# JettHuang/jet-pbrt

Hardware: AMD Instinct MI355X
Metric: Msamples/sec (whole node) + per-pixel L2 vs CPU ref, cornell_box 1024spp (higher is better)
Workload: dtype f32

## Files before the change

### jet-pbrt_amd/__init__.py

```python
import ctypes as C
import os

PKG_DIR = os.path.dirname(os.path.abspath(__file__))
REPO_DIR = os.path.dirname(PKG_DIR)
HIP_LIB_PATH = os.environ.get("JETPBRT_AMD_LIB") or os.path.join(PKG_DIR, "csrc", "libjetpbrt_amd.so")
HOST_LIB_PATH = os.path.join(PKG_DIR, "host", "libjetpbrt_host.so")
CLI_PATH = os.path.join(PKG_DIR, "host", "jetpbrt")

JP_MAT_PARAM_STRIDE = 16
JP_SAMPLER_STOCK_MT19937, JP_SAMPLER_COUNTER, JP_SAMPLER_DEBUG = 0, 1, 2
JP_OK = 0

_fp = C.POINTER(C.c_float)
_ip = C.POINTER(C.c_int32)


class JpCamera(C.Structure):
    _fields_ = [("pos", C.c_float * 3), ("front", C.c_float * 3), ("right", C.c_float * 3), ("up", C.c_float * 3),
                ("res_x", C.c_float), ("res_y", C.c_float)]


class JpScene(C.Structure):
    _fields_ = [
        ("camera", JpCamera),
# ... 1053 lines not shown
        v = tri_vn if isinstance(tri_vn, JpVertexNormals) else vertex_normals(tri_vn)
        self._check(self.lib.jp_set_vertex_normals(self.h, C.byref(v)))

    def normal_info(self):
        i = JpNormalInfo()
        i.struct_bytes = C.sizeof(JpNormalInfo)
        self._check(self.lib.jp_get_normal_info(self.h, C.byref(i)))
        return i

    def set_normal_maps(self, maps):
        self._check(self.lib.jp_set_normal_maps(self.h, None if maps is None else C.byref(maps)))

    def normal_map_info(self):
        i = JpNormalMapInfo()
        i.struct_bytes = C.sizeof(JpNormalMapInfo)
        self._check(self.lib.jp_get_normal_map_info(self.h, C.byref(i)))
        return i

    def set_texture_sampling(self, sampling):
        self._check(self.lib.jp_set_texture_sampling(self.h, None if sampling is None else C.byref(sampling)))

    def texture_sampling_info(self):
        i = JpTexSamplingInfo()
        i.struct_bytes = C.sizeof(JpTexSamplingInfo)
        self._check(self.lib.jp_get_texture_sampling_info(self.h, C.byref(i)))
        return i

    def shading_normal(self, origin, direction, tmin, tmax):
        import numpy as np
        n = origin.shape[0]
        o = np.ascontiguousarray(origin, np.float32); d = np.ascontiguousarray(direction, np.float32)
        t0 = np.ascontiguousarray(tmin, np.float32); t1 = np.ascontiguousarray(tmax, np.float32)
        prim = np.zeros(n, np.int32); ng = np.zeros((n, 3), np.float32); ns = np.zeros((n, 3), np.float32)
        p = lambda a: a.ctypes.data_as(C.c_void_p)
        self._check(self.lib.jp_shading_normal(self.h, n, p(o), p(d), p(t0), p(t1), p(prim), p(ng), p(ns)))
        return prim, ng, ns

    def synchronize(self):
        self._check(self.lib.jp_synchronize(self.h))

    def set_profiling(self, on):
        self._check(self.lib.jp_set_profiling(self.h, 1 if on else 0))

    def counters(self):
        c = JpCounters()
        self._check(self.lib.jp_get_counters(self.h, C.byref(c)))
        return c

    def build_info(self):
        b = JpBuildInfo()
        self._check(self.lib.jp_get_build_info(self.h, C.byref(b)))
        return b

    def read_table(self, which):
        return _read_table(lambda out, cap, n: self.lib.jp_read_scene_table(self.h, _table_index(which), out, cap, n))

    def tree_info(self):
        i = JpTreeInfo()
        i.struct_bytes = C.sizeof(JpTreeInfo)
        self._check(self.lib.jp_get_tree_info(self.h, C.byref(i)))
        return i

    def trace(self, origin, direction, tmin, tmax):
        import numpy as np
        n = origin.shape[0]
        o = np.ascontiguousarray(origin, np.float32); d = np.ascontiguousarray(direction, np.float32)
        t0 = np.ascontiguousarray(tmin, np.float32); t1 = np.ascontiguousarray(tmax, np.float32)
        hit = np.zeros(n, np.int32); t = np.zeros(n, np.float32); prim = np.zeros(n, np.int32); nrm = np.zeros((n, 3), np.float32)
        p = lambda a: a.ctypes.data_as(C.c_void_p)
        self._check(self.lib.jp_trace(self.h, n, p(o), p(d), p(t0), p(t1), p(hit), p(t), p(prim), p(nrm)))
        return hit, t, prim, nrm

    def occluded(self, origin, direction, tmin, tmax):
        import numpy as np
        n = origin.shape[0]
        o = np.ascontiguousarray(origin, np.float32); d = np.ascontiguousarray(direction, np.float32)
        t0 = np.ascontiguousarray(tmin, np.float32); t1 = np.ascontiguousarray(tmax, np.float32)
        occ = np.zeros(n, np.int32); walk = C.c_int32(-1)
        p = lambda a: a.ctypes.data_as(C.c_void_p)
        self._check(self.lib.jp_occluded(self.h, n, p(o), p(d), p(t0), p(t1), p(occ), C.byref(walk)))
        return occ, int(walk.value)

    def bsdf(self, desc, normal, wo, wi, u):
        import numpy as np
        n = normal.shape[0]
        a = [np.ascontiguousarray(x, np.float32) for x in (normal, wo, wi, u)]
        out = dict(f=np.zeros((n, 3), np.float32), pdf=np.zeros(n, np.float32), sf=np.zeros((n, 3), np.float32), swi=np.zeros((n, 3), np.float32),
                   spdf=np.zeros(n, np.float32), sflags=np.zeros(n, np.int32))
        p = lambda x: x.ctypes.data_as(C.c_void_p)
        self._check(self.lib.jp_bsdf(self.h, C.byref(desc), n, p(a[0]), p(a[1]), p(a[2]), p(a[3]), p(out["f"]), p(out["pdf"]), p(out["sf"]), p(out["swi"]), p(out["spdf"]), p(out["sflags"])))
        return out

    def close(self):
        if self.h:
            self.lib.jp_destroy_context(self.h)
            self.h = C.c_void_p()

    def __del__(self):
        try:
            self.close()
        except Exception:
            pass


from . import scenes
from . import distributed
# ... 1 lines not shown
```

### jet-pbrt_amd/csrc/jp_device.h

```cpp
#pragma once
#include <hip/hip_runtime.h>
#include <stdint.h>
#include "jetpbrt_amd.h"
#include "jp_counter_rng.h"

#define JP_BLOCK 256
#define JP_STACK_DEPTH 32

namespace jp
{
struct V3 { float x, y, z; };
__device__ __forceinline__ V3 mk(float x, float y, float z) { V3 v; v.x = x; v.y = y; v.z = z; return v; }
__device__ __forceinline__ V3 operator+(V3 a, V3 b) { return mk(a.x + b.x, a.y + b.y, a.z + b.z); }
__device__ __forceinline__ V3 operator-(V3 a, V3 b) { return mk(a.x - b.x, a.y - b.y, a.z - b.z); }
__device__ __forceinline__ V3 operator-(V3 a) { return mk(-a.x, -a.y, -a.z); }
__device__ __forceinline__ V3 operator*(V3 a, float s) { return mk(a.x * s, a.y * s, a.z * s); }
__device__ __forceinline__ V3 operator*(float s, V3 a) { return mk(a.x * s, a.y * s, a.z * s); }
__device__ __forceinline__ V3 operator/(V3 a, float s) { return mk(a.x / s, a.y / s, a.z / s); }
__device__ __forceinline__ V3 cmul(V3 a, V3 b) { return mk(a.x * b.x, a.y * b.y, a.z * b.z); }
__device__ __forceinline__ V3 cdiv(V3 a, V3 b) { return mk(a.x / b.x, a.y / b.y, a.z / b.z); }
__device__ __forceinline__ V3 splat(float v) { return mk(v, v, v); }
__device__ __forceinline__ V3 csqrt(V3 a) { return mk(sqrtf(a.x), sqrtf(a.y), sqrtf(a.z)); }
__device__ __forceinline__ float dot(V3 a, V3 b) { return a.x * b.x + a.y * b.y + a.z * b.z; }
__device__ __forceinline__ float len2(V3 a) { return a.x * a.x + a.y * a.y + a.z * a.z; }
// ... 253 lines not shown
	    : "+v"(mask), "=&s"(saved) : "v"(a), "v"(b), "s"(bits) : "vcc", "scc");
}

template <bool kInfTmax>
__device__ __forceinline__ unsigned int flat_boxes_lean(const float4* flat_g, int n_flat, V3 o, V3 d, float tmin, float tmax)
{
	ConstFPtr flat = (ConstFPtr)flat_g;
	const float ix = __builtin_amdgcn_rcpf(d.x), iy = __builtin_amdgcn_rcpf(d.y), iz = __builtin_amdgcn_rcpf(d.z);
	unsigned int mask = 0;
	#define JP_FLAT_BOX(i) \
	{ \
		const float x0 = (flat[8 * (i) + 0] - o.x) * ix, x1 = (flat[8 * (i) + 4] - o.x) * ix; \
		const float y0 = (flat[8 * (i) + 1] - o.y) * iy, y1 = (flat[8 * (i) + 5] - o.y) * iy; \
		const float z0 = (flat[8 * (i) + 2] - o.z) * iz, z1 = (flat[8 * (i) + 6] - o.z) * iz; \
		const float tn = fmaxf(fmaxf(fminf(x0, x1), fminf(y0, y1)), fmaxf(fminf(z0, z1), tmin)); \
		const float fxy = fminf(fmaxf(x0, x1), fmaxf(y0, y1)), fz = fmaxf(z0, z1); \
		const float tf = kInfTmax ? fminf(fxy, fz) : fminf(fxy, fminf(fz, tmax)); \
		or_bits_if_le(mask, tn, tf * 1.000002f, __float_as_uint(flat[8 * (i) + 3])); \
	}
	int i0 = 0;
	for (; i0 + 4 <= n_flat; i0 += 4)
	{
		#pragma unroll
		for (int u = 0; u < 4; u++) JP_FLAT_BOX(i0 + u)
	}
	for (; i0 < n_flat; i0++) JP_FLAT_BOX(i0)
	#undef JP_FLAT_BOX
	return mask;
}

template <bool kAnyHit, bool k64, int kS, typename F = FeatAll, typename PrimPtr>
__device__ __forceinline__ int flat_prims(typename FlatMask<k64>::type mask, PrimPtr prims, V3 o, V3 d, float tmin, float& tmax)
{
	int hit = -1;
#ifdef JP_DBG_FLAT_P1ONLY
	mask = mask == (typename FlatMask<k64>::type)0x12345677u ? 1u : 0u;
#endif
	while (mask)
	{
		const int p = (k64 ? __ffsll((unsigned long long)mask) : __ffs((int)mask)) - 1;
		mask &= mask - 1;
		if (prim_hit<kS, F>(prims, p, o, d, tmin, tmax)) { hit = p; if (kAnyHit) return hit; }
	}
	return hit;
}

template <bool kAnyHit, int kS, typename F = FeatAll, bool kInfTmax = false, typename PrimPtr>
__device__ __forceinline__ int traverse_flat(const float4* flat_g, int n_flat, int n_prims, PrimPtr prims, V3 o, V3 d, float tmin, float& tmax)
{
	if constexpr (!F::curved)
		if (n_prims <= 32) return flat_prims<kAnyHit, false, kS, F>(flat_boxes_lean<kInfTmax>(flat_g, n_flat, o, d, tmin, tmax), prims, o, d, tmin, tmax);
	if (n_prims > 32) return flat_prims<kAnyHit, true, kS, F>(flat_boxes<true>(flat_g, n_flat, o, d, tmin, tmax), prims, o, d, tmin, tmax);
	return flat_prims<kAnyHit, false, kS, F>(flat_boxes<false>(flat_g, n_flat, o, d, tmin, tmax), prims, o, d, tmin, tmax);
}

template <bool kAnyHit, typename PrimPtr>
__device__ __forceinline__ int traverse_wide(const uint4* __restrict__ wide, PrimPtr prims, V3 o, V3 d, float tmin, float& tmax, unsigned int* stack)
{
	const float ix = 1.0f / d.x, iy = 1.0f / d.y, iz = 1.0f / d.z;
	const unsigned int octinv = 7u - ((d.x < 0 ? 1u : 0u) | (d.y < 0 ? 2u : 0u) | (d.z < 0 ? 4u : 0u));
	unsigned int ngx = 0, ngy = 0x80000000u;
	int hit = -1, sp = 0;
	for (;;)
	{
		unsigned int tgx = 0, tgy = 0;
		if (ngy > 0x00ffffffu)
		{
			const unsigned int bit = 31u - (unsigned int)__clz((int)ngy);
			ngy &= ~(1u << bit);
			if (ngy > 0x00ffffffu) { stack[(2 * sp) * JP_BLOCK] = ngx; stack[(2 * sp + 1) * JP_BLOCK] = ngy; sp++; }
			const unsigned int slot = (bit - 24u) ^ octinv;
			const unsigned int rel = (unsigned int)__popc(ngy & 0xffu & ~(0xffffffffu << slot));
			const unsigned int idx = ngx + rel;
			const uint4 q0 = wide[5 * idx + 0], q1 = wide[5 * idx + 1], q2 = wide[5 * idx + 2], q3 = wide[5 * idx + 3], q4 = wide[5 * idx + 4];
			const float sx = __uint_as_float(((q0.w & 0xffu) ) << 23), sy = __uint_as_float(((q0.w >> 8) & 0xffu) << 23), sz = __uint_as_float(((q0.w >> 16) & 0xffu) << 23);
			const float px = __uint_as_float(q0.x) - o.x, py = __uint_as_float(q0.y) - o.y, pz = __uint_as_float(q0.z) - o.z;
			unsigned int hm = 0;
			#pragma unroll
			for (int i = 0; i < 8; i++)
			{
				const int sh = 8 * (i & 3);
				const unsigned int m = ((i < 4 ? q1.z : q1.w) >> sh) & 0xffu;
				const float lx = (float)(((i < 4 ? q2.x : q2.y) >> sh) & 0xffu), ly = (float)(((i < 4 ? q2.z : q2.w) >> sh) & 0xffu), lz = (float)(((i < 4 ? q3.x : q3.y) >> sh) & 0xffu);
				const float hx = (float)(((i < 4 ? q3.z : q3.w) >> sh) & 0xffu), hy = (float)(((i < 4 ? q4.x : q4.y) >> sh) & 0xffu), hz = (float)(((i < 4 ? q4.z : q4.w) >> sh) & 0xffu);
				const float x0 = fmaf(lx, sx, px) * ix, x1 = fmaf(hx, sx, px) * ix;
				const float y0 = fmaf(ly, sy, py) * iy, y1 = fmaf(hy, sy, py) * iy;
				const float z0 = fmaf(lz, sz, pz) * iz, z1 = fmaf(hz, sz, pz) * iz;
				const float tn = fmaxf(fmaxf(fminf(x0, x1), fminf(y0, y1)), fmaxf(fminf(z0, z1), tmin));
				const float tf = fminf(fminf(fmaxf(x0, x1), fmaxf(y0, y1)), fminf(fmaxf(z0, z1), tmax));
				if (m != 0u && tn <= tf * 1.000002f)
				{
					const bool inner = (m & 0x18u) == 0x18u;
					const unsigned int bits = inner ? 1u : (m >> 5), at = inner ? 24u + ((m & 7u) ^ octinv) : (m & 31u);
					hm |= bits << at;
				}
			}
			ngx = q1.x; ngy = (hm & 0xff000000u) | (q0.w >> 24);
			tgx = q1.y; tgy = hm & 0x00ffffffu;
		}
		while (tgy)
		{
			const int j = __ffs((int)tgy) - 1;
			tgy &= tgy - 1;
			if (prim_hit<4>(prims, (int)tgx + j, o, d, tmin, tmax)) { hit = (int)tgx + j; if (kAnyHit) return hit; }
		}
		if (ngy <= 0x00ffffffu)
// ... 287 lines not shown
```

### jet-pbrt_amd/csrc/jp_kernels.hip

```cpp
#include "jp_common.h"
#include "jp_tex.h"
#include "jp_normals.h"
#include "jp_normal_map.h"
#include "jp_env.h"
#include "jp_mis.h"
#include "jp_lens.h"
#include "jp_xbsdf.h"
#include "jp_film.h"

#include <cstdio>
#include <cstring>
#include <string>
#include <vector>
#include <algorithm>
#include <cmath>
#include <mutex>
#include <thread>
#include "jp_devmem.h"
#include "jp_lbvh.h"
#include "jp_ploc.h"

struct NoLens {};
template <bool kLens> struct LensArg { typedef NoLens type; };
template <> struct LensArg<true> { typedef JpLensPlan type; };
// ... 692 lines not shown
	{
		const unsigned int e = rbase + j;
#ifdef JP_TRAV_TIMING
		JP_TT(1);
		asm volatile("s_waitcnt vmcnt(0)" ::: "memory");
		JP_TT(2);
#endif
		const float4 so = so_n; float4 sd = sd_n;
		if (j + JP_BLOCK < E) { so_n = q.sh_o[e + JP_BLOCK]; sd_n = q.sh_d[e + JP_BLOCK]; }
		const int packed = __float_as_int(so.w);
		const int slot = packed & ((1 << rc.slot_bits) - 1), n = (int)((unsigned int)packed >> rc.slot_bits);
		if (n == 0) continue;
		bool any = false;
		const float4 L = q.lacc[slot];
		V3 a = mk(L.x, L.y, L.z);
		for (int k = 0; k < n; k++)
		{
			const float4 c4 = q.sh_c[(size_t)k * q.cap + e];
			float tmax = sd.w;
			const V3 dir = xyz(sd);
			if (k + 1 < n) sd = q.sh_d[(size_t)(k + 1) * q.cap + e];
			JP_TT(3);
#ifdef JP_TRAV_TIMING
			int hit;
			if constexpr (kMode == 2)
			{
				unsigned int m;
				if constexpr (F::curved) m = flat_boxes<false>(sc.flat, sc.n_flat, xyz(so), dir, 0.001f, tmax);
				else m = flat_boxes_lean<false>(sc.flat, sc.n_flat, xyz(so), dir, 0.001f, tmax);
				JP_TT(4);
				hit = flat_prims<true, false, 5, F>(m, acc.prims, xyz(so), dir, 0.001f, tmax);
				JP_TT(5);
			}
			else hit = acc.template trace<true>(sc, xyz(so), dir, 0.001f, tmax);
#else
			const int hit = acc.template trace<true>(sc, xyz(so), dir, 0.001f, tmax);
#endif
			rays++;
			if (hit >= 0) occ++;
			else { a = a + xyz(c4); any = true; }
			JP_TT(6);
		}
		if (any) q.lacc[slot] = make_float4(a.x, a.y, a.z, 0.f);
		JP_TT(7);
	}
#ifdef JP_TRAV_TIMING
	JP_TT(1);
	if ((threadIdx.x & 63) == 0) { for (int i = 0; i < 8; i++) atomicAdd(&g_shade_t[i], t_acc[i]); atomicAdd(&g_shade_t[15], 1ull); }
#endif
	for (int off = 32; off > 0; off >>= 1) { rays += __shfl_down(rays, off); occ += __shfl_down(occ, off); }
	if ((threadIdx.x & 63) == 0) { if (rays) atomicAdd(&cnt->shadow, (unsigned long long)rays); if (occ) atomicAdd(&cnt->shadow_occ, (unsigned long long)occ); }
}

template <int kMode, bool kAnyHit, bool kVote>
__device__ __forceinline__ void persist_turn(Walker<kMode>& w, const SceneView& sc, const WalkStack& stack, bool pool)
{
	const int nh = __popcll(__ballot(!w.done && w.heavy())), nl = __popcll(__ballot(!w.done && !w.heavy()));
	const bool heavyTurn = kVote ? nh > nl : w.heavy();
	if (kVote) { JP_TURN(heavyTurn ? 3 : 0, 1); JP_TURN(heavyTurn ? 4 : 1, heavyTurn ? nh : nl); JP_TURN(heavyTurn ? 5 : 2, nh + nl); if (!pool) { JP_TURN(8, 1); JP_TURN(9, nh + nl); JP_TURN(10, heavyTurn ? nh : nl); } }
	if (!w.done && (w.heavy() == heavyTurn)) w.template step<kAnyHit>(sc, stack);
}
__device__ __forceinline__ unsigned int lane_rank(unsigned long long m) { return __builtin_amdgcn_mbcnt_hi((unsigned int)(m >> 32), __builtin_amdgcn_mbcnt_lo((unsigned int)m, 0u)); }

#ifndef JP_CERT_WAVES
#define JP_CERT_WAVES 8
#endif
template <int kMode, int kRefill, bool kVote>
__global__ void __launch_bounds__(JP_BLOCK, (kMode == 6 ? JP_CERT_WAVES : 8)) k_extend_persist(SceneView sc, Queues q, int cur_q, int stack_cap, int* spill, DevCounters* cnt)
{
	__shared__ unsigned int s_next;
	const WalkStack stack = { (int*)s_dyn + threadIdx.x, spill + blockIdx.x * JP_BLOCK + threadIdx.x, (kMode == 4 || kMode == 6) ? stack_cap - 1 : stack_cap, gridDim.x * JP_BLOCK };
	const unsigned int b = blockIdx.x, n = q.blk_q[cur_q][b], rbase = b * q.R;
	if (b == 0 && threadIdx.x == 0) { cnt->closest += cnt->n_queue[cur_q]; cnt->n_queue[cur_q ^ 1] = 0; cnt->n_shadow = 0; }
	if (threadIdx.x == 0) s_next = 0;
	__syncthreads();
	const int lane = threadIdx.x & 63;
	Walker<kMode> w; w.done = true; w.hit = -1; w.tmax = JP_INF;
	unsigned int ridx = 0xffffffffu, h = 0;
	bool pool = n > 0;
	for (;;)
	{
		const unsigned long long idle = __ballot(w.done);
		const int nidle = __popcll(idle);
		if (nidle == 64 || (pool && nidle >= kRefill))
		{
			if (w.done && ridx != 0xffffffffu)
			{
				int hp = w.hit;
				if constexpr (kMode == 6) { if (!w.certain(sc)) hp = -2; }
				q.hit[rbase + ridx] = make_float2(w.tmax, __int_as_float(hp)); h += hp >= 0 ? 1u : 0u; ridx = 0xffffffffu;
			}
			if (!pool) break;
			const int first = __ffsll((long long)idle) - 1;
			unsigned int start = 0;
			if (lane == first) start = atomicAdd(&s_next, (unsigned int)nidle);
			start = __shfl(start, first);
			{ constexpr bool kAnyHit = false; (void)kAnyHit; JP_TURN(6, 1); JP_TURN(7, nidle); }
			pool = start + (unsigned int)nidle < n;
			if (w.done)
			{
				const unsigned int my = start + lane_rank(idle);
				if (my < n)
				{
					const float4 ro = q.ray_o[cur_q][rbase + my], rd = q.ray_d[cur_q][rbase + my];
					w.start(xyz(ro), xyz(rd), 0.001f, JP_INF);
					if constexpr (kMode == 6) w.mark_origin(sc);
// ... 485 lines not shown
```

### jet-pbrt_amd/csrc/jp_render.h

```cpp
#pragma once
namespace
{
enum { CLS_EXTEND = 0, CLS_SHADE = 1, CLS_SHADOW = 2, CLS_OTHER = 3, CLS_PATH = 4, CLS_NORMAL = 5, CLS_NMAP = 6, CLS_TEXEL = 7 };

int lens_plan_of(const JpContext* c, JpLensPlan& lp)
{
	std::memset(&lp, 0, sizeof(lp));
	if (!c->lens_on) return JP_OK;
	if (jp_lens_make_plan(&c->plan.sv.cam, &c->lens, &lp) != 0) return fail(JP_ERR_INVALID_ARGUMENT, "jp_set_lens: the uploaded camera's right / up vectors have no finite positive length");
	return JP_OK;
}

void free_queues(JpContext* c) { c->qb = QueueBufs(); c->cap = 0; c->planes_alloc = 0; c->blk_alloc = 0; }

int ensure_queues(JpContext* c, unsigned int cap, int planes, unsigned int nblocks)
{
	if (c->cap >= cap && c->planes_alloc >= planes && c->blk_alloc >= nblocks) return JP_OK;
	cap = std::max(cap, c->cap); planes = std::max(planes, c->planes_alloc); nblocks = std::max(nblocks, c->blk_alloc);
	free_queues(c);
	auto alloc = [](DevBuf& b, auto*& p, size_t bytes) { return reserve(b, p, bytes) == hipSuccess; };
	Queues& q = c->q; QueueBufs& qb = c->qb; bool ok = true;
	for (int b = 0; b < 2 && ok; b++) ok = alloc(qb.ray_o[b], q.ray_o[b], (size_t)cap * 16) && alloc(qb.ray_d[b], q.ray_d[b], (size_t)cap * 16) && alloc(qb.beta[b], q.beta[b], (size_t)cap * 16)
	                                       && alloc(qb.blk_q[b], q.blk_q[b], (size_t)nblocks * 4);
	ok = ok && alloc(qb.hit, q.hit, (size_t)cap * 8) && alloc(qb.lacc, q.lacc, (size_t)cap * 16) && alloc(qb.sh_o, q.sh_o, (size_t)cap * 16)
// ... 59 lines not shown
	const int nbands = (rp->height + s.band - 1) / s.band;
	s.local_rows = 0;
	for (int b = s.index; b < nbands; b += s.count) s.local_rows += std::min(s.band, rp->height - b * s.band);
	s.lane_rows = 0;
	for (int g0 = lane_index * lane_group; g0 < s.local_rows; g0 += lane_count * lane_group) s.lane_rows += std::min(lane_group, s.local_rows - g0);
	return JP_OK;
}

inline bool refill_walks(const ScenePlan& p) { return p.persist && (p.trav_mode == 0 || p.trav_mode == 3 || p.trav_mode == 5); }
inline int refill_row(const ScenePlan& p) { return p.persist >= 32 ? 2 : (p.persist >= 16 ? 1 : 0); }
inline int extend_depth(const ScenePlan& p) { return (p.trav_mode == 5 ? p.cert : p.use_q4) ? p.stack_depth_q4 : p.stack_depth; }
inline int shadow_depth(const ScenePlan& p) { return (p.trav_mode == 5 ? p.cert : p.q4_shadow) ? p.stack_depth_q4 : (p.trav_mode == 3 ? (int)(p.lds_bytes_shadow / (JP_BLOCK * sizeof(int))) : p.stack_depth); }
inline int deepest_walk(const ScenePlan& p) { return std::max(std::max(p.stack_depth, p.stack_depth_q4), p.trav_mode == 3 ? (int)(p.lds_bytes_shadow / (JP_BLOCK * sizeof(int))) : 0); }
inline size_t spill_need(const ScenePlan& p, int deep, unsigned int G) { return deep >= p.stack_lds_words ? (size_t)(deep - p.stack_lds_words + 1) * G * JP_BLOCK : 1; }

inline bool flat_shapes_only(int shape_mask) { return (shape_mask & ~((1 << JP_SHAPE_TRIANGLE) | (1 << JP_SHAPE_RECTANGLE))) == 0; }
inline bool lean_traversal(const ScenePlan& p, bool generic) { return !generic && p.trav_mode == 2 && flat_shapes_only(p.shape_mask); }
inline bool lean_shading(const ScenePlan& p, bool generic)
{
	const int delta_classes = (2 << JP_MAT_MIRROR) | (2 << JP_MAT_GLASS) | (2 << JP_MAT_PLASTIC);
	return !generic && p.shade_prims_in_lds && p.stage_nee && flat_shapes_only(p.shape_mask) && (p.light_mask & ~(1 << JP_LIGHT_AREA)) == 0
	    && flat_shapes_only(p.light_shape_mask) && (p.class_mask & delta_classes) == 0;
}

typedef void (*ExtendKernel)(SceneView, Queues, int, int, DevCounters*);
typedef void (*ExtendRefillKernel)(SceneView, Queues, int, int, int*, DevCounters*);
struct ExtendLaunch { ExtendRefillKernel refill; ExtendKernel plain; size_t lds; int words; };
template <int M> ExtendRefillKernel extend_refill(const ScenePlan& p)
{
	static const ExtendRefillKernel k[3][2] = { { k_extend_persist<M, 8, false>, k_extend_persist<M, 8, true> }, { k_extend_persist<M, 16, false>, k_extend_persist<M, 16, true> }, { k_extend_persist<M, 32, false>, k_extend_persist<M, 32, true> } };
	return k[refill_row(p)][p.vote];
}
ExtendLaunch extend_kernel(const ScenePlan& p, bool generic)
{
	if (lean_traversal(p, generic)) return { nullptr, k_extend<2, FeatFlat>, p.lds_bytes, p.stack_depth };
	if (!refill_walks(p)) return { nullptr, p.trav_mode == 5 ? k_extend<5> : (p.trav_mode == 2 ? k_extend<2> : (p.trav_mode == 1 ? k_extend<1> : k_extend<0>)), p.lds_bytes, p.stack_depth };
	const int words = std::min(extend_depth(p), p.stack_lds_words);
	const ExtendRefillKernel k = p.trav_mode == 5 ? (p.cert ? extend_refill<6>(p) : extend_refill<5>(p)) : (p.use_q4 ? extend_refill<4>(p) : extend_refill<0>(p));
	return { k, nullptr, (size_t)words * JP_BLOCK * sizeof(int), words };
}

typedef void (*ShadowKernel)(SceneView, Queues, RenderConst, int, DevCounters*);
typedef void (*ShadowRefillKernel)(SceneView, Queues, RenderConst, int, int*, DevCounters*);
struct ShadowLaunch { ShadowRefillKernel refill; ShadowKernel plain; size_t lds; int words; bool cert_fell_back; };
template <int M> ShadowRefillKernel shadow_refill(const ScenePlan& p)
{
	static const ShadowRefillKernel k[3][2] = { { k_shadow_persist<M, 8, false>, k_shadow_persist<M, 8, true> }, { k_shadow_persist<M, 16, false>, k_shadow_persist<M, 16, true> }, { k_shadow_persist<M, 32, false>, k_shadow_persist<M, 32, true> } };
	return k[refill_row(p)][p.vote];
}
ShadowLaunch shadow_kernel(const ScenePlan& p, unsigned int R, bool generic)
{
	const int words = std::min(shadow_depth(p), p.stack_lds_words);
	const size_t plds = (size_t)words * JP_BLOCK * sizeof(int) + (((size_t)R * p.n_planes + 31) / 32) * 4 * (p.cert ? 2 : 1);
	if (lean_traversal(p, generic)) return { nullptr, k_shadow<2, FeatFlat>, p.lds_bytes, p.stack_depth, p.cert };
	if (!refill_walks(p) || plds > 64 * 1024)
		return { nullptr, p.trav_mode == 3 ? k_shadow<3> : (p.trav_mode == 5 ? k_shadow<5> : (p.trav_mode == 2 ? k_shadow<2> : (p.trav_mode == 1 ? k_shadow<1> : k_shadow<0>))), p.trav_mode == 3 ? p.lds_bytes_shadow : p.lds_bytes, p.stack_depth, p.cert };
	const ShadowRefillKernel k = p.trav_mode == 5 ? (p.cert ? shadow_refill<6>(p) : shadow_refill<5>(p)) : (p.q4_shadow ? shadow_refill<4>(p) : (p.trav_mode == 3 ? shadow_refill<3>(p) : shadow_refill<0>(p)));
	return { k, nullptr, plds, words, false };
}

typedef void (*ShadeKernel)(SceneView, Queues, RenderConst, int, DevCounters*);
typedef void (*ShadeTexKernel)(SceneView, Queues, RenderConst, int, DevCounters*, TexView);
struct ShadeKernels { ShadeKernel plain; ShadeTexKernel tex; };
template <bool kTab, bool kPrims, bool kStage> ShadeKernels shade_row(bool sort)
{
	ShadeKernels k = { sort ? k_shade<kTab, kPrims, kStage, true> : k_shade<kTab, kPrims, kStage, false>, sort ? k_shade_tex<kTab, kPrims, kStage, true> : k_shade_tex<kTab, kPrims, kStage, false> };
	return k;
}
ShadeKernels shade_kernels(const ScenePlan& p, bool generic)
{
	if (lean_shading(p, generic))
	{
		ShadeKernels k = shade_row<true, true, true>(p.shade_sort);
		k.plain = p.shade_sort ? k_shade<true, true, true, true, FeatLean> : k_shade<true, true, true, false, FeatLean>;
#ifndef JP_NO_ONE_SWEEP
		if (p.shade_sort && !p.has_null_material) k.plain = k_shade_lean_one;
#endif
		return k;
	}
	if (p.shade_prims_in_lds) return p.stage_nee ? shade_row<true, true, true>(p.shade_sort) : shade_row<true, true, false>(p.shade_sort);
	if (p.tables_in_lds) return p.stage_nee ? shade_row<true, false, true>(p.shade_sort) : shade_row<true, false, false>(p.shade_sort);
	return shade_row<false, false, false>(p.shade_sort);
}

typedef void (*ShadePickKernel)(SceneView, Queues, RenderConst, int, DevCounters*, PickView);
typedef void (*ShadePickTexKernel)(SceneView, Queues, RenderConst, int, DevCounters*, TexView, PickView);
struct ShadePickKernels { ShadePickKernel plain; ShadePickTexKernel tex; };
ShadePickKernels shade_pick_kernels(const ScenePlan& p);
typedef void (*ShadeEnvKernel)(SceneView, Queues, RenderConst, int, DevCounters*, PickView, EnvView);
typedef void (*ShadeEnvTexKernel)(SceneView, Queues, RenderConst, int, DevCounters*, TexView, PickView, EnvView);
struct ShadeEnvKernels { ShadeEnvKernel plain; ShadeEnvTexKernel tex; };
ShadeEnvKernels shade_env_kernels(const ScenePlan& p);
typedef void (*ShadeMisKernel)(SceneView, Queues, RenderConst, int, DevCounters*, PickView, MisView);
typedef void (*ShadeMisTexKernel)(SceneView, Queues, RenderConst, int, DevCounters*, TexView, PickView, MisView);
typedef void (*ShadeMisEnvKernel)(SceneView, Queues, RenderConst, int, DevCounters*, PickView, EnvView, MisView);
typedef void (*ShadeMisEnvTexKernel)(SceneView, Queues, RenderConst, int, DevCounters*, TexView, PickView, EnvView, MisView);
struct ShadeMisKernels { ShadeMisKernel pick; ShadeMisTexKernel pick_tex; ShadeMisEnvKernel env; ShadeMisEnvTexKernel env_tex; };
ShadeMisKernels shade_mis_kernels(const ScenePlan& p);
struct SmoothKernels
{
	void (*normal)(SceneView, Queues, int, NormView);
	void (*normal_map)(SceneView, Queues, int, NormView, NMapView);
	void (*plain)(SceneView, Queues, RenderConst, int, DevCounters*, NormView);
	void (*tex)(SceneView, Queues, RenderConst, int, DevCounters*, TexView, NormView);
	void (*pick)(SceneView, Queues, RenderConst, int, DevCounters*, PickView, NormView);
	void (*pick_tex)(SceneView, Queues, RenderConst, int, DevCounters*, TexView, PickView, NormView);
// ... 594 lines not shown
	const OccludedLaunch ok = occluded_kernel(c->plan, c->opt.trace_walk, c->opt.reserved[0] == 1);
	if (walk_out) *walk_out = ok.walk;
	if (n == 0) return JP_OK;
	HIP_TRY(hipSetDevice(c->device));
	DevBuf b_o, b_d, b_t0, b_t1, b_occ;
	float *d_o, *d_d, *d_t0, *d_t1; int* d_occ;
	HIP_TRY(reserve(b_o, d_o, (size_t)n * 12)); HIP_TRY(reserve(b_d, d_d, (size_t)n * 12)); HIP_TRY(reserve(b_t0, d_t0, (size_t)n * 4)); HIP_TRY(reserve(b_t1, d_t1, (size_t)n * 4));
	HIP_TRY(reserve(b_occ, d_occ, (size_t)n * 4));
	HIP_TRY(hipMemcpyAsync(d_o, origin, (size_t)n * 12, hipMemcpyHostToDevice, c->stream)); HIP_TRY(hipMemcpyAsync(d_d, dir, (size_t)n * 12, hipMemcpyHostToDevice, c->stream));
	HIP_TRY(hipMemcpyAsync(d_t0, tmin, (size_t)n * 4, hipMemcpyHostToDevice, c->stream)); HIP_TRY(hipMemcpyAsync(d_t1, tmax, (size_t)n * 4, hipMemcpyHostToDevice, c->stream));
	const int grid = std::min(c->n_cus * 8, (n + JP_BLOCK - 1) / JP_BLOCK);
	hipLaunchKernelGGL(ok.occluded, dim3(grid), dim3(JP_BLOCK), ok.lds, c->stream, c->plan.sv, ok.depth, n, d_o, d_d, d_t0, d_t1, d_occ);
	HIP_TRY(hipGetLastError());
	HIP_TRY(hipMemcpyAsync(occluded, d_occ, (size_t)n * 4, hipMemcpyDeviceToHost, c->stream));
	HIP_TRY(hipStreamSynchronize(c->stream));
	return JP_OK;
}

int jp_get_texture_info(JpContext* c, JpTextureInfo* out)
{
	if (!c || !out) return fail(JP_ERR_INVALID_ARGUMENT, "jp_get_texture_info: null argument");
	if (out->struct_bytes < (int32_t)sizeof(int32_t)) return fail(JP_ERR_INVALID_ARGUMENT, "jp_get_texture_info: set JpTextureInfo.struct_bytes to sizeof(JpTextureInfo)");
	JpTextureInfo i; std::memset(&i, 0, sizeof(i));
	i.n_textures = c->plan.textured ? c->n_textures : 0; i.n_textured_materials = c->n_tex_mats; i.texel_bytes_device = c->texel_bytes; i.textured_last_render = c->last_textured;
	const size_t n = std::min((size_t)out->struct_bytes, sizeof(i));
	i.struct_bytes = (int32_t)n;
	std::memcpy(out, &i, n);
	return JP_OK;
}

int jp_surface(JpContext* c, int32_t n, const float* origin, const float* dir, const float* tmin, const float* tmax, int32_t* prim, float* uv, float* albedo)
{
	if (!c || n < 0 || !origin || !dir || !tmin || !tmax || !prim || !uv || !albedo) return fail(JP_ERR_INVALID_ARGUMENT, "jp_surface: null argument");
	if (!c->plan.have_scene) return fail(JP_ERR_NO_SCENE, "jp_surface: no scene uploaded");
	if (n == 0) return JP_OK;
	HIP_TRY(hipSetDevice(c->device));
	DevBuf b_in, b_uv, b_a, b_prim; float *d_in, *d_uv, *d_a; int* d_prim;
	HIP_TRY(reserve(b_in, d_in, (size_t)n * 32)); HIP_TRY(reserve(b_uv, d_uv, (size_t)n * 8)); HIP_TRY(reserve(b_a, d_a, (size_t)n * 12)); HIP_TRY(reserve(b_prim, d_prim, (size_t)n * 4));
	float *d_o = d_in, *d_d = d_in + 3 * (size_t)n, *d_t0 = d_in + 6 * (size_t)n, *d_t1 = d_in + 7 * (size_t)n;
	HIP_TRY(hipMemcpyAsync(d_o, origin, (size_t)n * 12, hipMemcpyHostToDevice, c->stream)); HIP_TRY(hipMemcpyAsync(d_d, dir, (size_t)n * 12, hipMemcpyHostToDevice, c->stream));
	HIP_TRY(hipMemcpyAsync(d_t0, tmin, (size_t)n * 4, hipMemcpyHostToDevice, c->stream)); HIP_TRY(hipMemcpyAsync(d_t1, tmax, (size_t)n * 4, hipMemcpyHostToDevice, c->stream));
	const int grid = std::min(c->n_cus * 8, (n + JP_BLOCK - 1) / JP_BLOCK);
	const TraceLaunch tk = trace_kernel(c->plan, 0);
	hipLaunchKernelGGL(tk.surface, dim3(grid), dim3(JP_BLOCK), tk.lds, c->stream, c->plan.sv, c->plan.tv, tk.depth, n, d_o, d_d, d_t0, d_t1, d_prim, d_uv, d_a, c->plan.sm);
	HIP_TRY(hipGetLastError());
	HIP_TRY(hipMemcpyAsync(prim, d_prim, (size_t)n * 4, hipMemcpyDeviceToHost, c->stream)); HIP_TRY(hipMemcpyAsync(uv, d_uv, (size_t)n * 8, hipMemcpyDeviceToHost, c->stream));
	HIP_TRY(hipMemcpyAsync(albedo, d_a, (size_t)n * 12, hipMemcpyDeviceToHost, c->stream));
	HIP_TRY(hipStreamSynchronize(c->stream));
	return JP_OK;
}

}

#if defined(JP_SHADE_TIMING) || defined(JP_TRAV_TIMING)
extern "C" int jp_dbg_shade_timing(unsigned long long* out16)
{
	unsigned long long z[16] = { 0 };
	if (hipMemcpyFromSymbol(out16, HIP_SYMBOL(g_shade_t), sizeof(z)) != hipSuccess) return -1;
	if (hipMemcpyToSymbol(HIP_SYMBOL(g_shade_t), z, sizeof(z)) != hipSuccess) return -1;
	return 0;
}
#endif

#ifdef JP_WALK_STATS
extern "C" int jp_dbg_walk_stats(unsigned long long* out8)
{
	unsigned long long z[8] = { 0 };
	if (hipMemcpyFromSymbol(out8, HIP_SYMBOL(jp::g_walk_stats), sizeof(z)) != hipSuccess) return -1;
	if (hipMemcpyToSymbol(HIP_SYMBOL(jp::g_walk_stats), z, sizeof(z)) != hipSuccess) return -1;
	return 0;
}
extern "C" int jp_dbg_turn_stats(unsigned long long* out32)
{
	unsigned long long z[32] = { 0 };
	if (hipMemcpyFromSymbol(out32, HIP_SYMBOL(jp::g_turn_stats), sizeof(z)) != hipSuccess) return -1;
	if (hipMemcpyToSymbol(HIP_SYMBOL(jp::g_turn_stats), z, sizeof(z)) != hipSuccess) return -1;
	return 0;
}
#endif

#ifdef JP_PATH_TIMING
extern "C" int jp_dbg_path_timing(unsigned long long* out16)
{
	unsigned long long z[16] = { 0 };
	if (hipMemcpyFromSymbol(out16, HIP_SYMBOL(g_path_t), sizeof(z)) != hipSuccess) return -1;
	if (hipMemcpyToSymbol(HIP_SYMBOL(g_path_t), z, sizeof(z)) != hipSuccess) return -1;
	return 0;
}
#endif
```

Measured before the change: 3306.

## Trace shadow rays in pairs against flat BVH for small scenes

Adds a k_shadow_pair kernel that tests two shadow rays from the same origin together, sharing box loads and origin-relative offsets in the flat box test and sharing primitive loads and edge cross products in the primitive test. It is selected for lean-traversal scenes with at most 32 primitives and at least two light planes, which covers the cornell box. The aim is to amortise memory loads and setup arithmetic across rays. In exchange it raises register pressure and can lose some early exit, because the primitive loop continues until both rays resolve. A debug query for which shadow kernel is in use is also added.

Result: faster. 3381 (median of 6 runs) (+2.3%).

```diff
diff --git a/jet-pbrt_amd/__init__.py b/jet-pbrt_amd/__init__.py
--- a/jet-pbrt_amd/__init__.py
+++ b/jet-pbrt_amd/__init__.py
@@ -1129,6 +1129,13 @@
         self._check(self.lib.jp_get_build_info(self.h, C.byref(b)))
         return b
 
+    def shadow_kernel(self):
+        fn = self.lib.jp_dbg_shadow_kernel
+        fn.argtypes = [C.c_void_p, C.POINTER(C.c_int)]; fn.restype = C.c_int
+        which = C.c_int(-1)
+        self._check(fn(self.h, C.byref(which)))
+        return ("refill", "generic", "flat", "pair")[which.value]
+
     def read_table(self, which):
         return _read_table(lambda out, cap, n: self.lib.jp_read_scene_table(self.h, _table_index(which), out, cap, n))
 
diff --git a/jet-pbrt_amd/csrc/jp_device.h b/jet-pbrt_amd/csrc/jp_device.h
--- a/jet-pbrt_amd/csrc/jp_device.h
+++ b/jet-pbrt_amd/csrc/jp_device.h
@@ -329,6 +329,87 @@
 		if (n_prims <= 32) return flat_prims<kAnyHit, false, kS, F>(flat_boxes_lean<kInfTmax>(flat_g, n_flat, o, d, tmin, tmax), prims, o, d, tmin, tmax);
 	if (n_prims > 32) return flat_prims<kAnyHit, true, kS, F>(flat_boxes<true>(flat_g, n_flat, o, d, tmin, tmax), prims, o, d, tmin, tmax);
 	return flat_prims<kAnyHit, false, kS, F>(flat_boxes<false>(flat_g, n_flat, o, d, tmin, tmax), prims, o, d, tmin, tmax);
+}
+
+__device__ __forceinline__ void flat_boxes_lean_pair(const float4* flat_g, int n_flat, V3 o, V3 dA, V3 dB, float tmin, float tmaxA, float tmaxB, unsigned int& mA, unsigned int& mB)
+{
+	ConstFPtr flat = (ConstFPtr)flat_g;
+	const float ixA = __builtin_amdgcn_rcpf(dA.x), iyA = __builtin_amdgcn_rcpf(dA.y), izA = __builtin_amdgcn_rcpf(dA.z);
+	const float ixB = __builtin_amdgcn_rcpf(dB.x), iyB = __builtin_amdgcn_rcpf(dB.y), izB = __builtin_amdgcn_rcpf(dB.z);
+	unsigned int maskA = 0, maskB = 0;
+	#define JP_FLAT_BOX_RAY(mask, ix, iy, iz, tmax) \
+	{ \
+		const float x0 = sx0 * ix, x1 = sx1 * ix, y0 = sy0 * iy, y1 = sy1 * iy, z0 = sz0 * iz, z1 = sz1 * iz; \
+		const float tn = fmaxf(fmaxf(fminf(x0, x1), fminf(y0, y1)), fmaxf(fminf(z0, z1), tmin)); \
+		const float fxy = fminf(fmaxf(x0, x1), fmaxf(y0, y1)), fz = fmaxf(z0, z1); \
+		const float tf = fminf(fxy, fminf(fz, tmax)); \
+		or_bits_if_le(mask, tn, tf * 1.000002f, bits); \
+	}
+	#define JP_FLAT_BOX(i) \
+	{ \
+		const float sx0 = flat[8 * (i) + 0] - o.x, sx1 = flat[8 * (i) + 4] - o.x; \
+		const float sy0 = flat[8 * (i) + 1] - o.y, sy1 = flat[8 * (i) + 5] - o.y; \
+		const float sz0 = flat[8 * (i) + 2] - o.z, sz1 = flat[8 * (i) + 6] - o.z; \
+		const unsigned int bits = __float_as_uint(flat[8 * (i) + 3]); \
+		JP_FLAT_BOX_RAY(maskA, ixA, iyA, izA, tmaxA) \
+		JP_FLAT_BOX_RAY(maskB, ixB, iyB, izB, tmaxB) \
+	}
+	int i0 = 0;
+	for (; i0 + 4 <= n_flat; i0 += 4)
+	{
+		#pragma unroll
+		for (int u = 0; u < 4; u++) JP_FLAT_BOX(i0 + u)
+	}
+	for (; i0 < n_flat; i0++) JP_FLAT_BOX(i0)
+	#undef JP_FLAT_BOX
+	#undef JP_FLAT_BOX_RAY
+	mA = maskA; mB = maskB;
+}
+
+template <int kS, typename PrimPtr>
+__device__ __forceinline__ void flat_prims_pair(unsigned int mA, unsigned int mB, PrimPtr prims, V3 o, V3 dA, V3 dB, float tmin, float tmaxA, float tmaxB, bool& hitA, bool& hitB)
+{
+	bool hA = false, hB = false;
+	unsigned int todo = mA | mB;
+	while (todo)
+	{
+		const int p = __ffs((int)todo) - 1;
+		const unsigned int bit = todo & (0u - todo);
+		todo &= todo - 1;
+		const float4 g0 = prims[kS * p + 0], g1 = prims[kS * p + 1], g2 = prims[kS * p + 2], g3 = prims[kS * p + 3];
+		const V3 n = xyz(g3);
+		const V3 oa = xyz(g0) - o;
+		const float noa = dot(n, oa);
+		const float distA = noa / dot(n, dA), distB = noa / dot(n, dB);
+		const bool passA = (mA & bit) && (distA > tmin) && (distA < tmaxA);
+		const bool passB = (mB & bit) && (distB > tmin) && (distB < tmaxB);
+		if (passA || passB)
+		{
+			const V3 ob = xyz(g1) - o, oc = xyz(g2) - o;
+			const V3 v0 = cross(oc, ob), v1 = cross(ob, oa);
+			const float v0A = dot(v0, dA), v1A = dot(v1, dA), v0B = dot(v0, dB), v1B = dot(v1, dB);
+			bool inA, inB;
+			if (__float_as_int(g3.w) == JP_SHAPE_TRIANGLE)
+			{
+				const V3 v2 = cross(oa, oc);
+				const float v2A = dot(v2, dA), v2B = dot(v2, dB);
+				inA = ((v0A < 0) && (v1A < 0) && (v2A < 0)) || ((v0A >= 0) && (v1A >= 0) && (v2A >= 0));
+				inB = ((v0B < 0) && (v1B < 0) && (v2B < 0)) || ((v0B >= 0) && (v1B >= 0) && (v2B >= 0));
+			}
+			else
+			{
+				const V3 od = mk(g0.w, g1.w, g2.w) - o;
+				const V3 v2 = cross(oa, od), v3 = cross(od, oc);
+				const float v2A = dot(v2, dA), v3A = dot(v3, dA), v2B = dot(v2, dB), v3B = dot(v3, dB);
+				inA = ((v0A < 0) && (v1A < 0) && (v2A < 0) && (v3A < 0)) || ((v0A >= 0) && (v1A >= 0) && (v2A >= 0) && (v3A >= 0));
+				inB = ((v0B < 0) && (v1B < 0) && (v2B < 0) && (v3B < 0)) || ((v0B >= 0) && (v1B >= 0) && (v2B >= 0) && (v3B >= 0));
+			}
+			if (passA && inA) { hA = true; mA = 0; }
+			if (passB && inB) { hB = true; mB = 0; }
+			todo &= mA | mB;
+		}
+	}
+	hitA = hA; hitB = hB;
 }
 
 template <bool kAnyHit, typename PrimPtr>
diff --git a/jet-pbrt_amd/csrc/jp_kernels.hip b/jet-pbrt_amd/csrc/jp_kernels.hip
--- a/jet-pbrt_amd/csrc/jp_kernels.hip
+++ b/jet-pbrt_amd/csrc/jp_kernels.hip
@@ -768,6 +768,64 @@
 	if ((threadIdx.x & 63) == 0) { if (rays) atomicAdd(&cnt->shadow, (unsigned long long)rays); if (occ) atomicAdd(&cnt->shadow_occ, (unsigned long long)occ); }
 }
 
+__global__ void __launch_bounds__(JP_BLOCK, 6) k_shadow_pair(SceneView sc, Queues q, RenderConst rc, int depth, DevCounters* cnt)
+{
+	typedef FeatFlat F;
+	SceneAccess<2, F> acc(sc, depth);
+	const unsigned int b = blockIdx.x, E = q.blk_sh[b], rbase = b * q.R;
+	unsigned int rays = 0, occ = 0;
+	float4 so_n = make_float4(0, 0, 0, 0), sd_n = make_float4(0, 0, 1, 0), sd1_n = make_float4(0, 0, 1, 0);
+	if (threadIdx.x < E) { so_n = q.sh_o[rbase + threadIdx.x]; sd_n = q.sh_d[rbase + threadIdx.x]; sd1_n = q.sh_d[(size_t)q.cap + rbase + threadIdx.x]; }
+	for (unsigned int j = threadIdx.x; j < E; j += JP_BLOCK)
+	{
+		const unsigned int e = rbase + j;
+		const float4 so = so_n; float4 sd = sd_n, sd1 = sd1_n;
+		if (j + JP_BLOCK < E) { so_n = q.sh_o[e + JP_BLOCK]; sd_n = q.sh_d[e + JP_BLOCK]; sd1_n = q.sh_d[(size_t)q.cap + e + JP_BLOCK]; }
+		const int packed = __float_as_int(so.w);
+		const int slot = packed & ((1 << rc.slot_bits) - 1), n = (int)((unsigned int)packed >> rc.slot_bits);
+		if (n == 0) continue;
+		bool any = false;
+		const float4 L = q.lacc[slot];
+		V3 a = mk(L.x, L.y, L.z);
+		for (int k = 0; k < n; k += 2)
+		{
+			const bool two = k + 1 < n;
+			const float4 cA = q.sh_c[(size_t)k * q.cap + e];
+			float4 cB = make_float4(0, 0, 0, 0);
+			if (two) cB = q.sh_c[(size_t)(k + 1) * q.cap + e];
+			const float tmaxA = sd.w, tmaxB = two ? sd1.w : sd.w;
+			const V3 dA = xyz(sd), dB = two ? xyz(sd1) : xyz(sd);
+			if (k + 2 < n) sd = q.sh_d[(size_t)(k + 2) * q.cap + e];
+			if (k + 3 < n) sd1 = q.sh_d[(size_t)(k + 3) * q.cap + e];
+			unsigned int mA, mB;
+#ifdef JP_NO_PAIR_BOXES
+			mA = flat_boxes_lean<false>(sc.flat, sc.n_flat, xyz(so), dA, 0.001f, tmaxA);
+			mB = flat_boxes_lean<false>(sc.flat, sc.n_flat, xyz(so), dB, 0.001f, tmaxB);
+#else
+			flat_boxes_lean_pair(sc.flat, sc.n_flat, xyz(so), dA, dB, 0.001f, tmaxA, tmaxB, mA, mB);
+#endif
+			if (!two) mB = 0;
+			bool hitA, hitB;
+#ifdef JP_NO_PAIR_PRIMS
+			{ float tA = tmaxA, tB = tmaxB; hitA = flat_prims<true, false, 5, F>(mA, acc.prims, xyz(so), dA, 0.001f, tA) >= 0; hitB = flat_prims<true, false, 5, F>(mB, acc.prims, xyz(so), dB, 0.001f, tB) >= 0; }
+#else
+			flat_prims_pair<5>(mA, mB, acc.prims, xyz(so), dA, dB, 0.001f, tmaxA, tmaxB, hitA, hitB);
+#endif
+			rays += two ? 2u : 1u;
+			if (hitA) occ++;
+			else { a = a + xyz(cA); any = true; }
+			if (two)
+			{
+				if (hitB) occ++;
+				else { a = a + xyz(cB); any = true; }
+			}
+		}
+		if (any) q.lacc[slot] = make_float4(a.x, a.y, a.z, 0.f);
+	}
+	for (int off = 32; off > 0; off >>= 1) { rays += __shfl_down(rays, off); occ += __shfl_down(occ, off); }
+	if ((threadIdx.x & 63) == 0) { if (rays) atomicAdd(&cnt->shadow, (unsigned long long)rays); if (occ) atomicAdd(&cnt->shadow_occ, (unsigned long long)occ); }
+}
+
 template <int kMode, bool kAnyHit, bool kVote>
 __device__ __forceinline__ void persist_turn(Walker<kMode>& w, const SceneView& sc, const WalkStack& stack, bool pool)
 {
diff --git a/jet-pbrt_amd/csrc/jp_render.h b/jet-pbrt_amd/csrc/jp_render.h
--- a/jet-pbrt_amd/csrc/jp_render.h
+++ b/jet-pbrt_amd/csrc/jp_render.h
@@ -135,6 +135,9 @@
 {
 	const int words = std::min(shadow_depth(p), p.stack_lds_words);
 	const size_t plds = (size_t)words * JP_BLOCK * sizeof(int) + (((size_t)R * p.n_planes + 31) / 32) * 4 * (p.cert ? 2 : 1);
+#ifndef JP_NO_SHADOW_PAIR
+	if (lean_traversal(p, generic) && p.sv.n_prims <= 32 && p.n_planes >= 2) return { nullptr, k_shadow_pair, p.lds_bytes, p.stack_depth, p.cert };
+#endif
 	if (lean_traversal(p, generic)) return { nullptr, k_shadow<2, FeatFlat>, p.lds_bytes, p.stack_depth, p.cert };
 	if (!refill_walks(p) || plds > 64 * 1024)
 		return { nullptr, p.trav_mode == 3 ? k_shadow<3> : (p.trav_mode == 5 ? k_shadow<5> : (p.trav_mode == 2 ? k_shadow<2> : (p.trav_mode == 1 ? k_shadow<1> : k_shadow<0>))), p.trav_mode == 3 ? p.lds_bytes_shadow : p.lds_bytes, p.stack_depth, p.cert };
@@ -835,6 +838,15 @@
 
 }
 
+extern "C" int jp_dbg_shadow_kernel(JpContext* c, int* which_out)
+{
+	if (!c || !which_out) return fail(JP_ERR_INVALID_ARGUMENT, "jp_dbg_shadow_kernel: null argument");
+	if (!c->plan.have_scene) return fail(JP_ERR_NO_SCENE, "jp_dbg_shadow_kernel: no scene uploaded");
+	const ShadowLaunch sk = shadow_kernel(c->plan, c->q.R ? c->q.R : JP_BLOCK, c->opt.reserved[0] == 1);
+	*which_out = sk.refill ? 0 : (sk.plain == (ShadowKernel)k_shadow_pair ? 3 : (sk.plain == (ShadowKernel)k_shadow<2, FeatFlat> ? 2 : 1));
+	return JP_OK;
+}
+
 #if defined(JP_SHADE_TIMING) || defined(JP_TRAV_TIMING)
 extern "C" int jp_dbg_shade_timing(unsigned long long* out16)
 {
```
